# ayf7/cuauv-vision-pipeline

Hardware: NVIDIA B200
Metric: frames/sec at 2208x1242 (higher is better)
Workload: dtype u8

## Files before the change

cuauv_vision_pipeline_b200/csrc/api.cu:

```cuda
#include <math.h>
#include <stdarg.h>
#include <stdlib.h>

#include <map>
#include <mutex>
#include <string>
#include <vector>

#include "common.cuh"
#include "lab_tables.inc"

namespace bv {

int rcp_tables_check(bv_ctx *ctx);

static thread_local char g_error[512] = "";

void set_error(const char *fmt, ...) {
    va_list ap;
    va_start(ap, fmt);
    vsnprintf(g_error, sizeof(g_error), fmt, ap);
    va_end(ap);
}

// ... 118 lines not shown
    return n;
}

extern "C" void bv_balance_default(bv_balance_params *p) {
    if (!p) return;
    p->equalize_rgb = 1;
    p->rgb_contrast_correct = 0;
    p->hsv_contrast_correct = 1;
    p->hsi_contrast_correct = 0;
    p->rgb_extrema_clipping = 1;
    p->adaptive_cast_correction = 0;
    p->horizontal_blocks = 1;
    p->vertical_blocks = 1;
}

extern "C" int bv_create(int device, bv_ctx **out) {
    BV_REQUIRE(out, "out is NULL");
    *out = nullptr;
    int n = 0;
    cudaError_t e = cudaGetDeviceCount(&n);
    if (e != cudaSuccess || n == 0) {
        set_error("bv_create: no usable CUDA device (%s); this library has no CPU path",
                  e == cudaSuccess ? "device count is 0" : cudaGetErrorString(e));
        (void)cudaGetLastError();
        return BV_ERR_CUDA;
    }
    BV_REQUIRE(device >= 0 && device < n, "device index out of range");
    BV_CUDA(cudaSetDevice(device));
    bv_ctx *ctx = (bv_ctx *)calloc(1, sizeof(bv_ctx));
    if (!ctx) {
        set_error("bv_create: out of host memory");
        return BV_ERR_NOMEM;
    }
    ctx->device = device;
    cudaDeviceProp prop;
    if ((e = cudaGetDeviceProperties(&prop, device)) != cudaSuccess) {
        set_error("cudaGetDeviceProperties: %s", cudaGetErrorString(e));
        free(ctx);
        return BV_ERR_CUDA;
    }
    ctx->sm_count = prop.multiProcessorCount;
    if ((e = cudaStreamCreateWithFlags(&ctx->own_stream, cudaStreamNonBlocking)) != cudaSuccess) {
        set_error("cudaStreamCreate: %s", cudaGetErrorString(e));
        free(ctx);
        return BV_ERR_CUDA;
    }
    ctx->stream = ctx->own_stream;
    bool ok_aux = cudaStreamCreateWithFlags(&ctx->copy_in, cudaStreamNonBlocking) == cudaSuccess &&
                  cudaStreamCreateWithFlags(&ctx->copy_out, cudaStreamNonBlocking) == cudaSuccess;
    for (int i = 0; ok_aux && i < BV_MAX_CHUNKS; ++i)
        ok_aux = cudaEventCreateWithFlags(&ctx->ev_in[i], cudaEventDisableTiming) == cudaSuccess &&
                 cudaEventCreateWithFlags(&ctx->ev_done[i], cudaEventDisableTiming) == cudaSuccess;
    for (int i = 0; ok_aux && i < BV_MAX_SIDE; ++i)
        ok_aux = cudaStreamCreateWithFlags(&ctx->side[i], cudaStreamNonBlocking) == cudaSuccess &&
                 cudaEventCreateWithFlags(&ctx->ev_join[i], cudaEventDisableTiming) == cudaSuccess;
    ok_aux = ok_aux && cudaEventCreateWithFlags(&ctx->ev_fork, cudaEventDisableTiming) == cudaSuccess;
    for (int i = 0; ok_aux && i < BV_HOST_SLOTS; ++i)
        ok_aux = cudaEventCreateWithFlags(&ctx->ev_slot[i], cudaEventDisableTiming) == cudaSuccess;
    if (!ok_aux) {
        set_error("bv_create: stream/event creation failed: %s", cudaGetErrorString(cudaGetLastError()));
        bv_destroy(ctx);
        return BV_ERR_CUDA;
    }
    double pow_tab[256];
    for (int x = 0; x < 256; ++x) pow_tab[x] = pow((255. - x) / 255., 0.25);
    bool ok = cudaMalloc(&ctx->d_lab_gamma, sizeof(kLabGammaTab)) == cudaSuccess &&
              cudaMalloc(&ctx->d_lab_cbrt, sizeof(kLabCbrtTab) + sizeof(kLabToYF) + sizeof(kLabInvGammaTab)) == cudaSuccess &&
              cudaMalloc(&ctx->d_pow_quarter, sizeof(pow_tab)) == cudaSuccess &&
              cudaMemcpy(ctx->d_lab_gamma, kLabGammaTab, sizeof(kLabGammaTab), cudaMemcpyHostToDevice) == cudaSuccess &&
              cudaMemcpy(ctx->d_lab_cbrt, kLabCbrtTab, sizeof(kLabCbrtTab), cudaMemcpyHostToDevice) == cudaSuccess &&
              cudaMemcpy(ctx->d_lab_cbrt + kLabCbrtSize, kLabToYF, sizeof(kLabToYF), cudaMemcpyHostToDevice) == cudaSuccess &&
              cudaMemcpy(ctx->d_lab_cbrt + kLabCbrtSize + 512, kLabInvGammaTab, sizeof(kLabInvGammaTab), cudaMemcpyHostToDevice) == cudaSuccess &&
              cudaMemcpy(ctx->d_pow_quarter, pow_tab, sizeof(pow_tab), cudaMemcpyHostToDevice) == cudaSuccess;
    if (!ok) {
        set_error("bv_create: table upload failed: %s", cudaGetErrorString(cudaGetLastError()));
        bv_destroy(ctx);
        return BV_ERR_CUDA;
    }
    if (bv::rcp_tables_check(ctx) != BV_OK) {
        bv_destroy(ctx);
        return BV_ERR_UNSUPPORTED;
    }
    static const char *const opt_env[BV_OPT_COUNT] = {"BV_HIST_BPS", "BV_FINAL_BPS", "BV_SIDE_STREAMS", "BV_L2_CHUNK_MB",
                                                      "BV_NO_HUE_TABLE", "BV_CONTOUR_POOL_CHUNKS", "BV_FAST_TABLES", "BV_MORPH_VARIANT", "BV_NO_RCP_TABLES", "BV_FINAL_SV_TABLES", "BV_MORPH_WARPS"};
    for (int i = 0; i < BV_OPT_COUNT; ++i) {
        const char *v = getenv(opt_env[i]);
        ctx->opt[i] = v ? atoi(v) : 0;
    }
    *out = ctx;
    return BV_OK;
}

extern "C" int bv_set_option(bv_ctx *ctx, int option, int value) {
    BV_REQUIRE(ctx, "null context");
    BV_REQUIRE(option >= 0 && option < BV_OPT_COUNT, "unknown option");
    ctx->opt[option] = value > 0 ? value : 0;
    return BV_OK;
}

extern "C" void bv_destroy(bv_ctx *ctx) {
    if (!ctx) return;
    cudaSetDevice(ctx->device);
    if (ctx->own_stream) cudaStreamSynchronize(ctx->own_stream);
    if (ctx->prof) {
        ctx->stream = ctx->own_stream;
        bv_profile_enable(ctx, 0);
    }
    for (int i = 0; i < SCR_COUNT; ++i)
        if (ctx->scratch[i]) cudaFree(ctx->scratch[i]);
    if (ctx->d_lab_gamma) cudaFree(ctx->d_lab_gamma);
    if (ctx->d_lab_cbrt) cudaFree(ctx->d_lab_cbrt);
    if (ctx->d_pow_quarter) cudaFree(ctx->d_pow_quarter);
    if (ctx->lb_cache) free(ctx->lb_cache);
    if (ctx->d_luv_tab) cudaFree(ctx->d_luv_tab);
    if (ctx->d_bilinear_tab) cudaFree(ctx->d_bilinear_tab);
    if (ctx->d_ivl_flag) cudaFree(ctx->d_ivl_flag);
    for (int i = 0; i < BV_IVL_SLOTS; ++i)
        if (ctx->ivl[i].table) cudaFree(ctx->ivl[i].table);
    if (ctx->own_stream) cudaStreamDestroy(ctx->own_stream);
    if (ctx->copy_in) cudaStreamDestroy(ctx->copy_in);
    if (ctx->copy_out) cudaStreamDestroy(ctx->copy_out);
    for (int i = 0; i < BV_MAX_SIDE; ++i) {
        if (ctx->side[i]) cudaStreamDestroy(ctx->side[i]);
        if (ctx->ev_join[i]) cudaEventDestroy(ctx->ev_join[i]);
    }
    if (ctx->ev_fork) cudaEventDestroy(ctx->ev_fork);
    for (int i = 0; i < BV_HOST_SLOTS; ++i)
        if (ctx->ev_slot[i]) cudaEventDestroy(ctx->ev_slot[i]);
    for (int i = 0; i < BV_MAX_CHUNKS; ++i) {
        if (ctx->ev_in[i]) cudaEventDestroy(ctx->ev_in[i]);
        if (ctx->ev_done[i]) cudaEventDestroy(ctx->ev_done[i]);
    }
    (void)cudaGetLastError();
    free(ctx);
}

extern "C" int bv_sync(bv_ctx *ctx) {
    BV_REQUIRE(ctx, "null context");
    BV_CUDA(cudaSetDevice(ctx->device));
    BV_CUDA(cudaStreamSynchronize(ctx->stream));
    return BV_OK;
}

extern "C" void *bv_stream(bv_ctx *ctx) { return ctx ? (void *)ctx->stream : nullptr; }

extern "C" int bv_set_stream(bv_ctx *ctx, void *cuda_stream) {
    BV_REQUIRE(ctx, "null context");
    ctx->stream = cuda_stream ? (cudaStream_t)cuda_stream : ctx->own_stream;
    return BV_OK;
}

extern "C" uint64_t bv_launch_count(const bv_ctx *ctx) { return ctx ? ctx->launches : 0; }
```

cuauv_vision_pipeline_b200/csrc/balance.cu:

```cuda
#include <stdlib.h>

#include "balance.cuh"
#include "convert.cuh"

namespace bv {

int hsi_run(bv_ctx *ctx, uint8_t *bgr, int batch, size_t npx);

constexpr int kBalThreads = 256;
constexpr int kBalWarps = kBalThreads / 32;

__device__ __forceinline__ int constrain255(double v) {
    if (v < 0.0) return 0;
    if (v > 255.0) return 255;
    if (v != v) return 0;
    return (int)v;
}

__device__ __forceinline__ int uchar_cast(double v) {
    if (v != v || v >= 2147483648.0 || v <= -2147483649.0) return 0;
    return ((int)v) & 0xFF;
}

__device__ __forceinline__ void stat_sync() { asm volatile("bar.sync 1, 256;" ::: "memory"); }
// ... 515 lines not shown
    if (MODE == 1 || MODE == 2)
        for (int i = threadIdx.x; i < 768; i += blockDim.x) (&fs.lut[0][0])[i] = (&st[frame].lut_bgr[0][0])[i];
    if (MODE >= 2)
        for (int i = threadIdx.x; i < 512; i += blockDim.x) (&fs.lut_sv[0][0])[i] = (&st[frame].lut_sv[0][0])[i];
    fill_sv_tabs<SVT>(svt, st[frame].lut_sv);
    __syncthreads();
    const size_t foff = (size_t)frame * npx;
    const uint8_t *f = src + (size_t)frame * src_stride;
    const int vec_end = width - (width % 32);
    constexpr bool kOne = CvtTraits<CODE>::kOneChannel;
    constexpr bool kNeedX = (MODE >= 2) || CvtTraits<CODE>::kNeedsX;
    const RangeTest bd = make_range_test(out.lo, out.hi);
    const uint32_t stride = gridDim.x * blockDim.x;
    const uint32_t ngroups = VEC ? (uint32_t)(npx / 16) : 0u;
    const uint32_t height = (uint32_t)(npx / (size_t)width);
    const int wp2 = ((width + 31) / 32) * 2;
    for (uint32_t g = blockIdx.x * blockDim.x + threadIdx.x; g < ngroups; g += stride) {
        Px16 in;
        load_px16<false>(f, g, in);
        uint32_t y = 0, x0 = 0;
        if (kNeedX || (NEED_MASK && out.mask_bits)) {
            const uint32_t p0 = g * 16u;
            y = p0 / (uint32_t)width;
            x0 = p0 - y * (uint32_t)width;
        }
        Px16 ob, oc;
        uint32_t q[4] = {0, 0, 0, 0};
        uint32_t bits = 0;
        uint32_t stg[4] = {0, 0, 0, 0};
#pragma unroll
        for (int k = 0; k < 12; ++k) ob.w[k] = oc.w[k] = 0;
        if (kNeedX && (int)x0 + 16 > vec_end)
            GroupBody<MODE, CODE, true, NEED_MASK, BAL, SVT, CVT, 0>::run(in, (int)x0, width, vec_end, fs, svt, tabs, bd, ob, oc, q, bits, stg);
        else
            GroupBody<MODE, CODE, false, NEED_MASK, BAL, SVT, CVT, 0>::run(in, (int)x0, width, vec_end, fs, svt, tabs, bd, ob, oc, q, bits, stg);
        if (BAL && out.balanced) store_px16(out.balanced + foff * 3, g, ob);
        if (CVT && out.converted) {
            if (kOne)
                st_stream(reinterpret_cast<uint4 *>(out.converted + foff) + g, make_uint4(q[0], q[1], q[2], q[3]));
            else
                store_px16(out.converted + foff * 3, g, oc);
        }
        if (NEED_MASK && out.mask) {
            uint32_t m[4];
#pragma unroll
            for (int k = 0; k < 4; ++k) {
                const uint32_t nib = (bits >> (4 * k)) & 0xF;
                m[k] = ((nib & 1) * 0xFFu) | (((nib >> 1) & 1) * 0xFF00u) | (((nib >> 2) & 1) * 0xFF0000u) |
                       (((nib >> 3) & 1) * 0xFF000000u);
            }
            st_stream(reinterpret_cast<uint4 *>(out.mask + foff) + g, make_uint4(m[0], m[1], m[2], m[3]));
        }
        if (NEED_MASK && out.mask_bits)
            out.mask_bits[((size_t)frame * height + y) * wp2 + (x0 >> 4)] = (uint16_t)bits;
        if (MODE == 3 && (src_stride & 127) == 0) discard_scratch_lines(f, g & ~31u, ngroups);
    }
    for (size_t p = (size_t)ngroups * 16 + (size_t)blockIdx.x * blockDim.x + threadIdx.x; p < npx; p += stride) {
        const int x = (int)(p % (size_t)width);
        const bool vec = x < vec_end;
        const uint32_t px = balance_px<MODE>(f[3 * p], f[3 * p + 1], f[3 * p + 2], vec, fs);
        const int b = (int)(px & 0xFF), gg = (int)((px >> 8) & 0xFF), r = (int)(px >> 16);
        if (out.balanced) {
            uint8_t *o = out.balanced + (foff + p) * 3;
            o[0] = (uint8_t)b;
            o[1] = (uint8_t)gg;
            o[2] = (uint8_t)r;
        }
        int o0, o1, o2;
        convert_px<CODE>(b, gg, r, vec, tabs, o0, o1, o2);
        if (out.converted) {
            if (kOne) {
                out.converted[foff + p] = (uint8_t)o0;
            } else {
                uint8_t *o = out.converted + (foff + p) * 3;
                o[0] = (uint8_t)o0;
                o[1] = (uint8_t)o1;
                o[2] = (uint8_t)o2;
            }
        }
        if (out.mask) out.mask[foff + p] = in_range_px<CODE>(o0, o1, o2, bd) ? 255 : 0;
    }
}

constexpr int kIvlEntries = 65536;
constexpr uint32_t kIvlBytes = kIvlEntries * 2;
constexpr int kIvlEmpty = 200;

__global__ void __launch_bounds__(256) ivl_build_kernel(uint16_t *__restrict__ table, int *__restrict__ bad, Bounds3 bd) {
    __shared__ int sdiv[256], hdiv[256];
    for (int i = threadIdx.x; i < 256; i += blockDim.x) {
        sdiv[i] = hsv_sdiv(i);
        hdiv[i] = hsv_hdiv(i);
    }
    __syncthreads();
    const RangeTest rt = make_range_test(bd.lo, bd.hi);
    const int lane = threadIdx.x & 31;
    const int pair = blockIdx.x * (blockDim.x >> 5) + (threadIdx.x >> 5);
    const int S = pair >> 8, V = pair & 255;
    auto passes = [&](int H) {
        const uint32_t p = hsv2bgr_packed(H, S, V, true);
        int h2, s2, v2;
        bgr2hsv((int)(p & 0xFF), (int)((p >> 8) & 0xFF), (int)(p >> 16), sdiv, hdiv, h2, s2, v2);
        return in_range_px<BV_BGR2HSV>(h2, s2, v2, rt);
    };
    int n_in = 0, n_rise = 0, first = 0;
    for (int it = 0; it < 6; ++it) {
        const int H = it * 32 + lane;
        bool in = false, rise = false;
        if (H < 180) {
            in = passes(H);
            rise = in && !passes(H == 0 ? 179 : H - 1);
        }
        const uint32_t bi = __ballot_sync(0xFFFFFFFFu, in), br = __ballot_sync(0xFFFFFFFFu, rise);
        n_in += __popc(bi);
        n_rise += __popc(br);
        if (br) first = it * 32 + __ffs(br) - 1;
    }
    if (lane == 0) {
        int lo = kIvlEmpty, span = 0;
        if (n_in == 180) {
            lo = 0;
            span = 179;
        } else if (n_in > 0) {
            if (n_rise != 1) atomicOr(bad, 1);
            const int last = (first + n_in - 1) % 180;
            lo = first;
            span = (last - first) & 0xFF;
        }
        table[pair] = (uint16_t)(lo | (span << 8));
    }
}

struct IvlSmem {
    uint16_t tab[kIvlEntries];
    uint64_t bar;
};

__global__ void __launch_bounds__(1024) ivl_compose_kernel(const uint16_t *__restrict__ table, const BalFrame *__restrict__ st,
                                                           uint16_t *__restrict__ composed) {
    __shared__ uint8_t lsv[2][256];
    const int frame = blockIdx.y;
    grid_dependency_wait();
    for (int i = threadIdx.x; i < 512; i += blockDim.x) (&lsv[0][0])[i] = (&st[frame].lut_sv[0][0])[i];
    __syncthreads();
    for (int idx = blockIdx.x * blockDim.x + threadIdx.x; idx < kIvlEntries; idx += gridDim.x * blockDim.x)
        composed[(size_t)frame * kIvlEntries + idx] = __ldg(table + (((uint32_t)lsv[0][idx & 255] << 8) | lsv[1][idx >> 8]));
}

__global__ void __launch_bounds__(1024, 1) mask_from_hsv_kernel(const uint8_t *__restrict__ hsv, size_t hsv_stride,
                                                                const BalFrame *__restrict__ st,
                                                                const uint16_t *__restrict__ table, size_t npx, int width,
                                                                BalOutputs out) {
    extern __shared__ __align__(128) unsigned char ivl_raw[];
    IvlSmem &sm = *reinterpret_cast<IvlSmem *>(ivl_raw);
    const int frame = blockIdx.y;
    if (threadIdx.x == 0) {
        mbar_init(&sm.bar, 1);
        mbar_expect_tx(&sm.bar, kIvlBytes);
        const unsigned char *mine = reinterpret_cast<const unsigned char *>(table + (size_t)frame * kIvlEntries);
        for (uint32_t o = 0; o < kIvlBytes; o += 32768u)
            bulk_g2s(reinterpret_cast<unsigned char *>(sm.tab) + o, mine + o, 32768u, &sm.bar);
    }
    const uint8_t *f = hsv + (size_t)frame * hsv_stride;
    const size_t foff = (size_t)frame * npx;
    const uint32_t stride = gridDim.x * blockDim.x, ngroups = (uint32_t)(npx / 16);
    const uint32_t height = (uint32_t)(npx / (size_t)width);
// ... 284 lines not shown
    return BV_OK
    switch (code) {
        case -1: BV_FT(-1);
        case BV_BGR2HSV: BV_FT(BV_BGR2HSV);
        case BV_BGR2LAB: BV_FT(BV_BGR2LAB);
        case BV_BGR2GRAY: BV_FT(BV_BGR2GRAY);
        case BV_BGR2YCRCB: BV_FT(BV_BGR2YCRCB);
        case BV_BGR2HLS: BV_FT(BV_BGR2HLS);
        default: set_error("stage: conversion code %d is not available in the fused pass", code); return BV_ERR_INVALID;
    }
#undef BV_FT
}

static int balance_run_tiled(bv_ctx *ctx, const uint8_t *src, int batch, int height, int width, const bv_balance_params &prm,
                             int cvt_code, const BalOutputs &out, BalFrame *st) {
    const int hb = prm.horizontal_blocks, vb = prm.vertical_blocks;
    if (hb < 1 || vb < 1 || width % hb || height % vb) {
        set_error("colour balance: horizontal/vertical_blocks must divide the frame (%dx%d into %dx%d tiles)", width, height, hb, vb);
        return BV_ERR_UNSUPPORTED;
    }
    const int n_tiles = hb * vb;
    if (n_tiles > 4096 || out.mask_bits) {
        set_error("colour balance: too many tiles, or bit-packed mask requested with tiling");
        return BV_ERR_UNSUPPORTED;
    }
    const size_t npx = (size_t)height * width;
    BV_TRY(ensure_scratch(ctx, SCR_BAL_TILES, sizeof(BalTile) * (size_t)batch * n_tiles));
    BalTile *tiles = (BalTile *)ctx->scratch[SCR_BAL_TILES];
    BV_CUDA(cudaMemsetAsync(tiles, 0, sizeof(BalTile) * (size_t)batch * n_tiles, ctx->stream));
    TileGeom tg{hb, vb, width / hb, height / vb, width, height};
    const size_t tile_px = (size_t)tg.bw * tg.bh;
    int bx = (int)((tile_px + kBalThreads * 16 - 1) / (kBalThreads * 16));
    const int cap = (ctx->sm_count * 8 + n_tiles * batch - 1) / (n_tiles * batch);
    if (bx > cap) bx = cap;
    if (bx < 1) bx = 1;
    dim3 grid(bx, n_tiles, batch);
    auto aligned4 = [](const void *q) { return (reinterpret_cast<uintptr_t>(q) & 3) == 0; };
    const bool vec4 = width % 4 == 0 && tg.bw % 4 == 0 && aligned4(src) && aligned4(out.balanced) && aligned4(out.converted) &&
                      aligned4(out.mask);
#define BV_HT(P)                                                                                                       \
    do {                                                                                                               \
        if (vec4)                                                                                                      \
            BV_LAUNCH(ctx, (hist_tiled_kernel<P, true>), grid, kBalThreads, 0, src, st, tiles, npx, tg, prm, ctx->d_pow_quarter); \
        else                                                                                                           \
            BV_LAUNCH(ctx, (hist_tiled_kernel<P, false>), grid, kBalThreads, 0, src, st, tiles, npx, tg, prm, ctx->d_pow_quarter); \
    } while (0)
    BV_HT(1);
    if (prm.hsv_contrast_correct) {
        BV_HT(2);
#undef BV_HT
        return dispatch_final_tiled<2>(ctx, src, st, tiles, grid, npx, tg, cvt_code, out, vec4);
    }
    return dispatch_final_tiled<1>(ctx, src, st, tiles, grid, npx, tg, cvt_code, out, vec4);
}

static int hist_blocks_per_sm(const bv_ctx *ctx) { return ctx->opt[BV_OPT_HIST_BPS] > 0 ? ctx->opt[BV_OPT_HIST_BPS] : (ctx->overlapped ? 2 : 4); }
static int final_blocks_per_sm(const bv_ctx *ctx) { return ctx->opt[BV_OPT_FINAL_BPS] > 0 ? ctx->opt[BV_OPT_FINAL_BPS] : (ctx->overlapped ? 2 : 8); }
static int side_streams(const bv_ctx *ctx) {
    const int v = ctx->opt[BV_OPT_SIDE_STREAMS] > 0 ? ctx->opt[BV_OPT_SIDE_STREAMS] : 4;
    return v > BV_MAX_SIDE ? BV_MAX_SIDE : v;
}
static size_t l2_chunk_bytes(const bv_ctx *ctx) { return (size_t)(ctx->opt[BV_OPT_L2_CHUNK_MB] > 0 ? ctx->opt[BV_OPT_L2_CHUNK_MB] : 33) << 20; }

static bool vec_ok(const void *p, size_t npx, int batch, int bytes_per_px) {
    (void)bytes_per_px;
    return p == nullptr || (host_aligned16(p) && (npx % 16 == 0 || batch == 1));
}

template <int MODE, int CODE>
static int launch_final(bv_ctx *ctx, const uint8_t *src, size_t src_stride, const BalFrame *st, int batch, size_t npx,
                        int width, const BalOutputs &out, bool vec) {
    int bpf = (ctx->sm_count * final_blocks_per_sm(ctx) + batch - 1) / batch;
    const size_t need = (npx / 16 + kBalThreads - 1) / kBalThreads;
    if ((size_t)bpf > need) bpf = (int)(need ? need : 1);
    dim3 grid(bpf, batch);
    const bool need_mask = out.mask || out.mask_bits;
#define BV_FINAL(V, M)                                                                                              \
    BV_LAUNCH_PDL(ctx, (final_kernel<MODE, CODE, V, M>), grid, kBalThreads, 0, src, src_stride, st, npx, width, out, \
                  ctx->d_lab_gamma, ctx->d_lab_cbrt)
#define BV_FINAL_NOBAL(M)                                                                                                     \
    BV_LAUNCH_PDL(ctx, (final_kernel<MODE, CODE, true, M, false>), grid, kBalThreads, 0, src, src_stride, st, npx, width, out, \
                  ctx->d_lab_gamma, ctx->d_lab_cbrt)
    const int svt = ctx->opt[BV_OPT_FINAL_SV_TABLES];
    if (MODE == 3 && CODE == BV_BGR2LAB && vec && !out.balanced && !need_mask && svt > 0) {
        if (svt == 1)
            BV_LAUNCH_PDL(ctx, (final_kernel<MODE, CODE, true, false, false, (MODE == 3 && CODE == BV_BGR2LAB) ? 1 : 0>), grid,
                          kBalThreads, 0, src, src_stride, st, npx, width, out, ctx->d_lab_gamma, ctx->d_lab_cbrt);
        else
            BV_LAUNCH_PDL(ctx, (final_kernel<MODE, CODE, true, false, false, (MODE == 3 && CODE == BV_BGR2LAB) ? 2 : 0>), grid,
                          kBalThreads, 0, src, src_stride, st, npx, width, out, ctx->d_lab_gamma, ctx->d_lab_cbrt);
    } else if (vec && CODE != -1 && !out.balanced && !out.converted && need_mask) {
        BV_LAUNCH_PDL(ctx, (final_kernel<MODE, CODE, true, true, false, 0, false>), grid, kBalThreads, 0, src, src_stride, st, npx,
                      width, out, ctx->d_lab_gamma, ctx->d_lab_cbrt);
    } else if (vec && CODE != -1 && !out.balanced) {
        if (need_mask) BV_FINAL_NOBAL(true); else BV_FINAL_NOBAL(false);
    } else if (vec) {
        if (need_mask) BV_FINAL(true, true); else BV_FINAL(true, false);
    } else {
        if (need_mask) BV_FINAL(false, true); else BV_FINAL(false, false);
    }
#undef BV_FINAL
#undef BV_FINAL_NOBAL
    return BV_OK;
}

template <int MODE>
static int dispatch_final(bv_ctx *ctx, const uint8_t *src, size_t src_stride, const BalFrame *st, int batch, size_t npx,
                          int width, int code, const BalOutputs &out, bool vec) {
    switch (code) {
        case -1: return launch_final<MODE, -1>(ctx, src, src_stride, st, batch, npx, width, out, vec);
        case BV_BGR2HSV: return launch_final<MODE, BV_BGR2HSV>(ctx, src, src_stride, st, batch, npx, width, out, vec);
        case BV_BGR2LAB: return launch_final<MODE, BV_BGR2LAB>(ctx, src, src_stride, st, batch, npx, width, out, vec);
        case BV_BGR2GRAY: return launch_final<MODE, BV_BGR2GRAY>(ctx, src, src_stride, st, batch, npx, width, out, vec);
        case BV_BGR2YCRCB: return launch_final<MODE, BV_BGR2YCRCB>(ctx, src, src_stride, st, batch, npx, width, out, vec);
        case BV_BGR2HLS: return launch_final<MODE, BV_BGR2HLS>(ctx, src, src_stride, st, batch, npx, width, out, vec);
        default: set_error("stage: conversion code %d is not available in the fused pass", code); return BV_ERR_INVALID;
    }
}

static bool all_vec(const uint8_t *src, const BalOutputs &out, size_t npx, int batch) {
    return vec_ok(src, npx, batch, 3) && vec_ok(out.balanced, npx, batch, 3) && vec_ok(out.converted, npx, batch, 3) &&
           vec_ok(out.mask, npx, batch, 1);
}

static int rcp_tables_usable(bv_ctx *ctx, bool *ok);

__global__ void rcp_tables_check_kernel(int *bad) {
    const int d = threadIdx.x;
    if (rint_quotient_rcp((float)(255 << kHsvShift), d) != hsv_sdiv(d) ||
        rint_quotient_rcp((float)((180 << kHsvShift) / 6), d) != hsv_hdiv(d))
        atomicOr(bad, 1);
}

int rcp_tables_check(bv_ctx *ctx) {
    bool ok = false;
    BV_TRY(rcp_tables_usable(ctx, &ok));
    if (ctx->rcp_state != 1) {
        set_error("bv_create: rcp.approx.f32 of this device does not reproduce OpenCV's sdiv / hdiv tables (library is built for sm_100a)");
        return BV_ERR_UNSUPPORTED;
    }
    return BV_OK;
}

static int rcp_tables_usable(bv_ctx *ctx, bool *ok) {
    if (ctx->rcp_state == 0) {
        if (!ctx->d_ivl_flag) BV_CUDA(cudaMalloc(&ctx->d_ivl_flag, sizeof(int)));
        BV_CUDA(cudaMemsetAsync(ctx->d_ivl_flag, 0, sizeof(int), ctx->stream));
        BV_LAUNCH(ctx, rcp_tables_check_kernel, 1, 256, 0, ctx->d_ivl_flag);
        int bad = 1;
        BV_CUDA(cudaMemcpyAsync(&bad, ctx->d_ivl_flag, sizeof(int), cudaMemcpyDeviceToHost, ctx->stream));
        BV_CUDA(cudaStreamSynchronize(ctx->stream));
        ctx->rcp_state = bad ? 2 : 1;
    }
    *ok = ctx->rcp_state == 1 && ctx->opt[BV_OPT_NO_RCP_TABLES] <= 0;
    return BV_OK;
}

static int fast_blocks_per_frame(const bv_ctx *ctx, int nf, size_t npx) {
    int bpf = (ctx->sm_count * 2 + nf - 1) / nf;
    const size_t need = (npx / 16 + kFastThreads - 1) / kFastThreads;
    if ((size_t)bpf > need) bpf = (int)(need ? need : 1);
    return bpf;
}

template <typename K>
static int enable_fast_smem(bv_ctx *ctx, K kernel, int bit, size_t bytes) {
    if (!(ctx->fast_attr_set & (1u << bit))) {
// ... 220 lines not shown
```

cuauv_vision_pipeline_b200/runtime.py:

```python
import threading

import numpy as np
import torch

from ._ffi import ffi, lib, check, BVError

CVT = {
    "bgr2hsv": lib.BV_BGR2HSV, "bgr2lab": lib.BV_BGR2LAB, "bgr2gray": lib.BV_BGR2GRAY,
    "bgr2ycrcb": lib.BV_BGR2YCRCB, "hsv2bgr": lib.BV_HSV2BGR, "bgr2hls": lib.BV_BGR2HLS,
    "gray2bgr": lib.BV_GRAY2BGR, "bgr2rgb": lib.BV_BGR2RGB, "lab2bgr": lib.BV_LAB2BGR, "bgr2luv": lib.BV_BGR2LUV,
}
MORPH = {"erode": lib.BV_MORPH_ERODE, "dilate": lib.BV_MORPH_DILATE, "open": lib.BV_MORPH_OPEN,
         "close": lib.BV_MORPH_CLOSE, "gradient": lib.BV_MORPH_GRADIENT}
THRESH = {"binary": lib.BV_THRESH_BINARY, "binary_inv": lib.BV_THRESH_BINARY_INV, "trunc": lib.BV_THRESH_TRUNC,
          "tozero": lib.BV_THRESH_TOZERO, "tozero_inv": lib.BV_THRESH_TOZERO_INV}

BLOB_DTYPE = np.dtype([(k, "<i8") for k in ("m00", "m10", "m01", "m20", "m11", "m02", "m30", "m21", "m12", "m03")] +
                      [(k, "<i4") for k in ("x0", "y0", "x1", "y1")])
assert BLOB_DTYPE.itemsize == ffi.sizeof("bv_blob")
CONTOUR_DTYPE = np.dtype([(k, "<i8") for k in ("a00", "a10", "a01")] +
                         [(k, "<i4") for k in ("x0", "y0", "x1", "y1", "start_x", "start_y", "n_points", "n_simple",
                                               "label", "external", "point_offset", "reserved")])
assert CONTOUR_DTYPE.itemsize == ffi.sizeof("bv_contour")
RRECT_DTYPE = np.dtype([(k, "<f4") for k in ("cx", "cy", "width", "height", "angle")] + [("valid", "<i4")])
assert RRECT_DTYPE.itemsize == ffi.sizeof("bv_rrect")
SHAPE_DTYPE = np.dtype([("arc_length", "<f8")] + [(k, "<f4") for k in ("circle_cx", "circle_cy", "circle_r")] +
                       [("rect", RRECT_DTYPE)] + [(k, "<i4") for k in ("n_hull", "n_approx", "approx_convex", "valid",
                                                                      "reserved")])
assert SHAPE_DTYPE.itemsize == ffi.sizeof("bv_shape")


def _u8ptr(t):
    return ffi.cast("uint8_t *", t.data_ptr()) if t is not None else ffi.NULL


class Context:

    def __init__(self, device=0):
        out = ffi.new("bv_ctx **")
        check(lib.bv_create(int(device), out))
        self._ctx = out[0]
        self.device = torch.device("cuda", int(device))
        self.torch_stream = torch.cuda.ExternalStream(int(ffi.cast("uintptr_t", lib.bv_stream(self._ctx))),
                                                      device=self.device)
        self._inflight = {}

    def close(self):
        if self._ctx is not None:
            for slot in list(self._inflight):
                lib.bv_stage_host_wait(self._ctx, slot)
            self._inflight.clear()
            lib.bv_destroy(self._ctx)
            self._ctx = None

    def __enter__(self):
        return self

    def __exit__(self, *exc):
        self.close()

    def __del__(self):
        try:
            self.close()
        except Exception:
            pass

    @property
    def handle(self):
        if self._ctx is None:
            raise BVError(-1, "context is closed")
        return self._ctx

    def sync(self):
        check(lib.bv_sync(self.handle))

    @property
    def launches(self):
        return int(lib.bv_launch_count(self.handle))

    OPTIONS = {"hist_bps": 0, "final_bps": 1, "side_streams": 2, "l2_chunk_mb": 3, "no_hue_table": 4, "contour_pool_chunks": 5,
               "fast_tables": 6, "morph_variant": 7, "no_rcp_tables": 8, "final_sv_tables": 9, "morph_warps": 10}

    def set_option(self, name, value):
        check(lib.bv_set_option(self.handle, self.OPTIONS[name], int(value)))

    def profile(self, on=True):
        check(lib.bv_profile_enable(self.handle, 1 if on else 0))

    def profile_dump(self):
        import json
        buf = ffi.new("char[]", 1 << 16)
        check(lib.bv_profile_dump(self.handle, buf, 1 << 16))
        return json.loads(ffi.string(buf).decode())

    def empty(self, shape, dtype=torch.uint8):
        with torch.cuda.stream(self.torch_stream):
            return torch.empty(shape, dtype=dtype, device=self.device)

    def upload(self, arr):
        if isinstance(arr, torch.Tensor):
            if arr.is_cuda:
                return arr.contiguous()
            src = arr.contiguous()
        else:
            src = torch.from_numpy(np.ascontiguousarray(arr))
        with torch.cuda.stream(self.torch_stream):
            return src.to(self.device, non_blocking=True)

    def download(self, t):
        with torch.cuda.stream(self.torch_stream):
            out = t.cpu()
        return out.numpy()

    @staticmethod
    def _bhw(t, channels=None):
        if t.dtype != torch.uint8 or not t.is_cuda or not t.is_contiguous():
            raise BVError(-1, "expected a contiguous CUDA uint8 tensor")
        if t.dim() == 2:
            return 1, t.shape[0], t.shape[1], 1
        if t.dim() == 3:
            if channels == 1:
                return t.shape[0], t.shape[1], t.shape[2], 1
            return 1, t.shape[0], t.shape[1], t.shape[2]
        if t.dim() == 4:
            return t.shape[0], t.shape[1], t.shape[2], t.shape[3]
        raise BVError(-1, "unsupported tensor rank")

    def _src(self, t):
        if t.dtype != torch.uint8 or t.device != self.device or not t.is_contiguous():
            raise BVError(-1, "expected a contiguous uint8 tensor on %s" % self.device)
        return t

    def cvt_color(self, src, code, split=False):
        code_i = CVT[code] if isinstance(code, str) else int(code)
        if code_i != lib.BV_GRAY2BGR:
            b, h, w, c = self._bhw(src)
        if code_i == lib.BV_GRAY2BGR:
            if src.dim() not in (2, 3):
                raise BVError(-1, "GRAY2BGR needs [H,W] or [B,H,W]")
            gb = 1 if src.dim() == 2 else src.shape[0]
            dst = self.empty(tuple(src.shape) + (3,))
            check(lib.bv_cvt_color(self.handle, _u8ptr(src), _u8ptr(dst), ffi.NULL, gb, src.shape[-2], src.shape[-1],
                                   code_i))
            return dst
        if c != 3:
            raise BVError(-1, "colour conversion needs a 3-channel image")
        one = code_i == lib.BV_BGR2GRAY
        lead = tuple(src.shape[:-1])
        dst = self.empty(lead if one else lead + (3,))
        planes = None
        if split and not one:
            planes = [self.empty(lead) for _ in range(3)]
            pp = ffi.new("uint8_t *[3]", [_u8ptr(p) for p in planes])
        else:
            pp = ffi.NULL
        check(lib.bv_cvt_color(self.handle, _u8ptr(src), _u8ptr(dst), pp, b, h, w, code_i))
        return (dst, planes) if split else dst

    @staticmethod
    def _cv_bounds(lo, hi, channels):
        lo = np.rint(np.atleast_1d(np.asarray(lo, dtype=np.float64))).astype(np.int64)
        hi = np.rint(np.atleast_1d(np.asarray(hi, dtype=np.float64))).astype(np.int64)
        if channels == 3:
            if lo.size == 1:
# ... 484 lines not shown
```

include/b200vision.h:

```cpp
#ifndef B200VISION_H
#define B200VISION_H

#include <stdbool.h>
#include <stddef.h>
#include <stdint.h>

#ifdef __cplusplus
extern "C" {
#endif

#define BV_VERSION 100

typedef struct bv_ctx bv_ctx;

typedef enum bv_status {
    BV_OK = 0,
    BV_ERR_INVALID = -1,
    BV_ERR_CUDA = -2,
    BV_ERR_UNSUPPORTED = -3,
    BV_ERR_NOMEM = -4,
    BV_ERR_CAPACITY = -5,
    BV_ERR_NOT_READY = -6
} bv_status;

// ... 4 lines not shown
    BV_BGR2YCRCB = 3,
    BV_HSV2BGR = 4,
    BV_BGR2HLS = 5,
    BV_GRAY2BGR = 6,
    BV_BGR2RGB = 7,
    BV_LAB2BGR = 8,
    BV_BGR2LUV = 9
} bv_cvt_code;

typedef enum bv_thresh_type {
    BV_THRESH_BINARY = 0,
    BV_THRESH_BINARY_INV = 1,
    BV_THRESH_TRUNC = 2,
    BV_THRESH_TOZERO = 3,
    BV_THRESH_TOZERO_INV = 4
} bv_thresh_type;

typedef enum bv_morph_op {
    BV_MORPH_ERODE = 0,
    BV_MORPH_DILATE = 1,
    BV_MORPH_OPEN = 2,
    BV_MORPH_CLOSE = 3,
    BV_MORPH_GRADIENT = 4
} bv_morph_op;

typedef struct bv_balance_params {
    int32_t equalize_rgb;
    int32_t rgb_contrast_correct;
    int32_t hsv_contrast_correct;
    int32_t hsi_contrast_correct;
    int32_t rgb_extrema_clipping;
    int32_t adaptive_cast_correction;
    int32_t horizontal_blocks;
    int32_t vertical_blocks;
} bv_balance_params;

typedef struct bv_balance_stats {
    int32_t bgr_min[3], bgr_max[3];
    double bgr_avg[3];
    int32_t dominant;
    int32_t s_min, s_max, v_min, v_max;
    int32_t degenerate;
} bv_balance_stats;

typedef struct bv_blob {
    int64_t m00, m10, m01, m20, m11, m02, m30, m21, m12, m03;
    int32_t x0, y0, x1, y1;
} bv_blob;

typedef struct bv_stage_desc {
    int32_t do_balance;
    bv_balance_params balance;
    int32_t cvt_code;
    uint8_t lo[3], hi[3];
    int32_t n_morph;
    int32_t morph_op[4];
    int32_t morph_kw[4], morph_kh[4];
    int32_t morph_iters[4];
    int32_t do_label;
} bv_stage_desc;

int bv_version(void);
const char *bv_last_error(void);
int bv_device_count(void);
int bv_create(int device, bv_ctx **out);
void bv_destroy(bv_ctx *ctx);
int bv_sync(bv_ctx *ctx);
void *bv_stream(bv_ctx *ctx);
int bv_set_stream(bv_ctx *ctx, void *cuda_stream);
uint64_t bv_launch_count(const bv_ctx *ctx);

enum {
    BV_OPT_HIST_BPS = 0,
    BV_OPT_FINAL_BPS = 1,
    BV_OPT_SIDE_STREAMS = 2,
    BV_OPT_L2_CHUNK_MB = 3,
    BV_OPT_NO_HUE_TABLE = 4,
    BV_OPT_CONTOUR_POOL_CHUNKS = 5,
    BV_OPT_FAST_TABLES = 6,
    BV_OPT_MORPH_VARIANT = 7,
    BV_OPT_NO_RCP_TABLES = 8,
    BV_OPT_FINAL_SV_TABLES = 9,
    BV_OPT_MORPH_WARPS = 10,
    BV_OPT_COUNT = 11
};
int bv_set_option(bv_ctx *ctx, int option, int value);
void bv_balance_default(bv_balance_params *p);
int bv_profile_enable(bv_ctx *ctx, int on);
int bv_profile_dump(bv_ctx *ctx, char *buf, size_t cap);

int bv_color_balance(bv_ctx *ctx, const uint8_t *src_dev, uint8_t *dst_dev, int batch, int height, int width,
                     const bv_balance_params *params, bv_balance_stats *stats_host);

int bv_cvt_color(bv_ctx *ctx, const uint8_t *src_dev, uint8_t *dst_dev, uint8_t *const *planes_dev, int batch,
                 int height, int width, int code);
int bv_in_range(bv_ctx *ctx, const uint8_t *src_dev, uint8_t *mask_dev, int batch, int height, int width,
                int channels, const uint8_t *lo_host, const uint8_t *hi_host);
int bv_threshold(bv_ctx *ctx, const uint8_t *src_dev, uint8_t *dst_dev, size_t n, int thresh, int maxval,
                 int type);
int bv_cvt_in_range(bv_ctx *ctx, const uint8_t *src_dev, uint8_t *mask_dev, int batch, int height, int width,
                    int code, const uint8_t *lo_host, const uint8_t *hi_host);
int bv_apply_lut(bv_ctx *ctx, const uint8_t *src_dev, uint8_t *dst_dev, size_t n_pixels, int channels,
                 const uint8_t *lut_host);

int bv_color_distance(bv_ctx *ctx, const uint8_t *const *planes_dev, size_t n, const double *color_host,
                      const double *weights_host, const int32_t *use_host, double max_dist_sq, uint8_t *mask_dev,
                      uint8_t *dist_dev);
int bv_color_distance_f32(bv_ctx *ctx, const uint8_t *const *planes_dev, size_t n, const double *color_host,
                          const double *weights_host, const int32_t *use_host, float *dists_dev);
int bv_select_kth_f32(bv_ctx *ctx, const float *values_dev, size_t n, size_t k, float *value_host);

int bv_morph(bv_ctx *ctx, const uint8_t *src_dev, uint8_t *dst_dev, int batch, int height, int width,
             int channels, int op, const uint8_t *se_host, int kw, int kh, int iterations);

int bv_canny(bv_ctx *ctx, const uint8_t *src_dev, uint8_t *dst_dev, int batch, int height, int width, int channels,
             double threshold1, double threshold2, int aperture_size, int l2_gradient);

int bv_label(bv_ctx *ctx, const uint8_t *mask_dev, int32_t *labels_dev, int batch, int height, int width,
             bv_blob *blobs_dev, int max_blobs, int32_t *n_blobs_dev);

typedef struct bv_contour {
    int64_t a00, a10, a01;
    int32_t x0, y0, x1, y1;
    int32_t start_x, start_y;
    int32_t n_points;
    int32_t n_simple;
    int32_t label;
    int32_t external;
    int32_t point_offset;
    int32_t reserved;
} bv_contour;

int bv_outer_contours(bv_ctx *ctx, const uint8_t *mask_dev, int batch, int height, int width,
                      bv_contour *contours_dev, int max_contours, int32_t *n_contours_dev, int32_t *points_dev,
                      int max_points, int32_t *n_points_dev);

typedef enum bv_retr_mode {
    BV_RETR_LIST = 1,
    BV_RETR_CCOMP = 2,
    BV_RETR_TREE = 3
} bv_retr_mode;
typedef enum bv_chain_approx {
    BV_CHAIN_APPROX_NONE = 1,
    BV_CHAIN_APPROX_SIMPLE = 2
} bv_chain_approx;
int bv_find_contours(bv_ctx *ctx, const uint8_t *mask_dev, int batch, int height, int width, int mode, int method,
                     bv_contour *contours_dev, int32_t *hierarchy_dev, int max_contours, int32_t *n_contours_dev,
                     int32_t *points_dev, int max_points, int32_t *n_points_dev);

typedef struct bv_rrect {
    float cx, cy, width, height, angle;
    int32_t valid;
} bv_rrect;
int bv_min_area_rects(bv_ctx *ctx, const bv_contour *contours_dev, const int32_t *n_contours_dev,
                      const int32_t *points_dev, int batch, int max_contours, int max_points, bv_rrect *rects_dev);

typedef struct bv_shape {
    double arc_length;
    float circle_cx, circle_cy, circle_r;
    bv_rrect rect;
    int32_t n_hull;
    int32_t n_approx;
    int32_t approx_convex;
    int32_t valid;
    int32_t reserved;
} bv_shape;
int bv_contour_shapes(bv_ctx *ctx, const bv_contour *contours_dev, const int32_t *n_contours_dev, int counts_per_frame,
// ... 79 lines not shown
```

Measured before the change: 74890.

## Add specialized HSV-to-Lab final kernel with shared-memory tables and byte-trick arithmetic

Adds a dedicated final_lab_kernel for the balance-then-BGR2LAB path without mask or balanced output. It copies gamma and cube-root tables into shared memory, turns HSV into BGR using float magic-number rounding and a packed prmt selector, and computes Lab with fixed-point integer matrices and table lookups. Output bytes are packed with byte_perm. It is the default route when width is a multiple of 32, and a new option falls back to the generic kernel. The cost is larger shared memory per block and a risk of rounding differences from the generic path.

```diff
diff --git a/cuauv_vision_pipeline_b200/csrc/api.cu b/cuauv_vision_pipeline_b200/csrc/api.cu
--- a/cuauv_vision_pipeline_b200/csrc/api.cu
+++ b/cuauv_vision_pipeline_b200/csrc/api.cu
@@ -224,7 +224,8 @@
         return BV_ERR_UNSUPPORTED;
     }
     static const char *const opt_env[BV_OPT_COUNT] = {"BV_HIST_BPS", "BV_FINAL_BPS", "BV_SIDE_STREAMS", "BV_L2_CHUNK_MB",
-                                                      "BV_NO_HUE_TABLE", "BV_CONTOUR_POOL_CHUNKS", "BV_FAST_TABLES", "BV_MORPH_VARIANT", "BV_NO_RCP_TABLES", "BV_FINAL_SV_TABLES", "BV_MORPH_WARPS"};
+                                                      "BV_NO_HUE_TABLE", "BV_CONTOUR_POOL_CHUNKS", "BV_FAST_TABLES", "BV_MORPH_VARIANT", "BV_NO_RCP_TABLES", "BV_FINAL_SV_TABLES", "BV_MORPH_WARPS",
+                                                      "BV_FINAL_LAB_GENERIC"};
     for (int i = 0; i < BV_OPT_COUNT; ++i) {
         const char *v = getenv(opt_env[i]);
         ctx->opt[i] = v ? atoi(v) : 0;
diff --git a/cuauv_vision_pipeline_b200/csrc/balance.cu b/cuauv_vision_pipeline_b200/csrc/balance.cu
--- a/cuauv_vision_pipeline_b200/csrc/balance.cu
+++ b/cuauv_vision_pipeline_b200/csrc/balance.cu
@@ -621,6 +621,85 @@
     }
 }
 
+constexpr unsigned long long kLabSel = 0x2114084100882014ull;
+
+struct LabSmem {
+    uint8_t lut_sv[2][256];
+    uint16_t gtab[kLabGammaSize];
+    uint16_t ctab[kLabCbrtSize];
+};
+
+__device__ __forceinline__ uint32_t lds_u16_at(const uint16_t *tab, uint32_t byte_off) {
+    return *reinterpret_cast<const uint16_t *>(reinterpret_cast<const uint8_t *>(tab) + byte_off);
+}
+
+template <int Q>
+__device__ __forceinline__ void put_byte2(uint32_t (&w)[12], uint32_t (&st)[4], uint32_t t) {
+    st[Q & 3] = t;
+    if constexpr ((Q & 3) == 3)
+        w[Q >> 2] = __byte_perm(__byte_perm(st[0], st[1], 0x0062u), __byte_perm(st[2], st[3], 0x0062u), 0x5410u);
+}
+
+template <int J>
+__device__ __forceinline__ void lab_group(const Px16 &in, const LabSmem &sm, Px16 &o, uint32_t (&stg)[4]) {
+    if constexpr (J < 16) {
+        constexpr int kH = 3 * J;
+        const float kTwo23 = 8388608.f, hscale = 6.f / 180.f, inv255 = 1.f / 255.f;
+        const uint32_t hb = __byte_perm(in.w[kH >> 2], 0x4B000000u, 0x7650u | (kH & 3));
+        const uint32_t sb = 0x4B000000u | sm.lut_sv[0][BV_GETB(in.w, kH + 1)];
+        const uint32_t vb = 0x4B000000u | sm.lut_sv[1][BV_GETB(in.w, kH + 2)];
+        const float h = __fmaf_rn(__uint_as_float(hb), hscale, -kTwo23 * hscale);
+        const float s = __fmaf_rn(__uint_as_float(sb), inv255, -kTwo23 * inv255);
+        const float v = __fmaf_rn(__uint_as_float(vb), inv255, -kTwo23 * inv255);
+        const uint32_t kb = __float_as_uint(__fadd_rz(h, kTwo23));
+        const float fm = fabsf(__fsub_rn(h, __fsub_rn(__uint_as_float(kb | 1u), kTwo23)));
+        const float ymax = __fmul_rn(v, 255.f);
+        const float ymin = __fmul_rn(__fmul_rn(v, __fsub_rn(1.f, s)), 255.f);
+        const float ymid = __fmul_rn(__fmul_rn(v, __fmaf_rn(-s, fm, 1.f)), 255.f);
+        const uint32_t amax = __float_as_uint(__fadd_rz(ymax, kTwo23));
+        const uint32_t amid = __float_as_uint(__fadd_rz(ymid, kTwo23));
+        const uint32_t amin = __float_as_uint(__fadd_rz(ymin, kTwo23));
+        const uint32_t sel = (uint32_t)(kLabSel >> (kb * 11u - 11u * 0x4B000000u));
+        uint32_t bgr;
+        asm("prmt.b32 %0, %1, %2, %3;" : "=r"(bgr) : "r"(__byte_perm(amax, amid, 0x1440u)), "r"(amin), "r"(sel));
+        const int B = (int)lds_u16_at(sm.gtab, (bgr << 1) & 0x1FEu);
+        const int G = (int)lds_u16_at(sm.gtab, (bgr >> 7) & 0x1FEu);
+        const int R = (int)lds_u16_at(sm.gtab, (bgr >> 15) & 0x1FEu);
+        const int fX = (int)lds_u16_at(sm.ctab, ((uint32_t)(R * 1777 + G * 1541 + B * 778 + 2048) >> 11) & ~1u);
+        const int fY = (int)lds_u16_at(sm.ctab, ((uint32_t)(R * 871 + G * 2929 + B * 296 + 2048) >> 11) & ~1u);
+        const int fZ = (int)lds_u16_at(sm.ctab, ((uint32_t)(R * 73 + G * 448 + B * 3575 + 2048) >> 11) & ~1u);
+        put_byte2<3 * J>(o.w, stg, (uint32_t)(592 * fY - 2 * (1336934 - (1 << 14))));
+        put_byte2<3 * J + 1>(o.w, stg, (uint32_t)(1000 * fX - 1000 * fY + 2 * ((128 << 15) + (1 << 14))));
+        put_byte2<3 * J + 2>(o.w, stg, (uint32_t)(400 * fY - 400 * fZ + 2 * ((128 << 15) + (1 << 14))));
+        lab_group<J + 1>(in, sm, o, stg);
+    }
+}
+
+__global__ void __launch_bounds__(kBalThreads) final_lab_kernel(const uint8_t *__restrict__ hsv, size_t hsv_stride,
+                                                                const BalFrame *__restrict__ st, size_t npx,
+                                                                uint8_t *__restrict__ lab, const uint16_t *__restrict__ g_gamma,
+                                                                const uint16_t *__restrict__ g_cbrt) {
+    __shared__ LabSmem sm;
+    for (int i = threadIdx.x; i < kLabGammaSize; i += blockDim.x) sm.gtab[i] = g_gamma[i];
+    for (int i = threadIdx.x; i < kLabCbrtSize; i += blockDim.x) sm.ctab[i] = g_cbrt[i];
+    const int frame = blockIdx.y;
+    grid_dependency_wait();
+    for (int i = threadIdx.x; i < 512; i += blockDim.x) (&sm.lut_sv[0][0])[i] = (&st[frame].lut_sv[0][0])[i];
+    __syncthreads();
+    const uint8_t *f = hsv + (size_t)frame * hsv_stride;
+    uint8_t *o = lab + (size_t)frame * npx * 3;
+    const uint32_t ngroups = (uint32_t)(npx / 16);
+    const uint32_t stride = gridDim.x * blockDim.x;
+    for (uint32_t g = blockIdx.x * blockDim.x + threadIdx.x; g < ngroups; g += stride) {
+        Px16 in, oc;
+        load_px16<false>(f, g, in);
+        uint32_t stg[4];
+        lab_group<0>(in, sm, oc, stg);
+        store_px16(o, g, oc);
+        if ((hsv_stride & 127) == 0) discard_scratch_lines(f, g & ~31u, ngroups);
+    }
+}
+
 constexpr int kIvlEntries = 65536;
 constexpr uint32_t kIvlBytes = kIvlEntries * 2;
 constexpr int kIvlEmpty = 200;
@@ -1071,7 +1150,11 @@
     BV_LAUNCH_PDL(ctx, (final_kernel<MODE, CODE, true, M, false>), grid, kBalThreads, 0, src, src_stride, st, npx, width, out, \
                   ctx->d_lab_gamma, ctx->d_lab_cbrt)
     const int svt = ctx->opt[BV_OPT_FINAL_SV_TABLES];
-    if (MODE == 3 && CODE == BV_BGR2LAB && vec && !out.balanced && !need_mask && svt > 0) {
+    if (MODE == 3 && CODE == BV_BGR2LAB && vec && width % 32 == 0 && out.converted && !out.balanced && !need_mask && svt <= 0 &&
+        ctx->opt[BV_OPT_FINAL_LAB_GENERIC] <= 0) {
+        BV_LAUNCH_PDL(ctx, final_lab_kernel, grid, kBalThreads, 0, src, src_stride, st, npx, out.converted, ctx->d_lab_gamma,
+                      ctx->d_lab_cbrt);
+    } else if (MODE == 3 && CODE == BV_BGR2LAB && vec && !out.balanced && !need_mask && svt > 0) {
         if (svt == 1)
             BV_LAUNCH_PDL(ctx, (final_kernel<MODE, CODE, true, false, false, (MODE == 3 && CODE == BV_BGR2LAB) ? 1 : 0>), grid,
                           kBalThreads, 0, src, src_stride, st, npx, width, out, ctx->d_lab_gamma, ctx->d_lab_cbrt);
diff --git a/cuauv_vision_pipeline_b200/runtime.py b/cuauv_vision_pipeline_b200/runtime.py
--- a/cuauv_vision_pipeline_b200/runtime.py
+++ b/cuauv_vision_pipeline_b200/runtime.py
@@ -79,7 +79,8 @@
         return int(lib.bv_launch_count(self.handle))
 
     OPTIONS = {"hist_bps": 0, "final_bps": 1, "side_streams": 2, "l2_chunk_mb": 3, "no_hue_table": 4, "contour_pool_chunks": 5,
-               "fast_tables": 6, "morph_variant": 7, "no_rcp_tables": 8, "final_sv_tables": 9, "morph_warps": 10}
+               "fast_tables": 6, "morph_variant": 7, "no_rcp_tables": 8, "final_sv_tables": 9, "morph_warps": 10,
+               "final_lab_generic": 11}
 
     def set_option(self, name, value):
         check(lib.bv_set_option(self.handle, self.OPTIONS[name], int(value)))
diff --git a/include/b200vision.h b/include/b200vision.h
--- a/include/b200vision.h
+++ b/include/b200vision.h
@@ -110,7 +110,8 @@
     BV_OPT_NO_RCP_TABLES = 8,
     BV_OPT_FINAL_SV_TABLES = 9,
     BV_OPT_MORPH_WARPS = 10,
-    BV_OPT_COUNT = 11
+    BV_OPT_FINAL_LAB_GENERIC = 11,
+    BV_OPT_COUNT = 12
 };
 int bv_set_option(bv_ctx *ctx, int option, int value);
 void bv_balance_default(bv_balance_params *p);
```

Result: no change. 74820 (median of 6 runs) (-0.1%).
